# tanqiu98/2G-GCN

Measured on AMD Instinct MI355X. Metric: clips/sec fwd+bwd, T=120 N=34 C=512, higher is better.
Workload: dtype fp32

## Files before the change

2g-gcn_amd/csrc/gemm_f32.hip:

```cpp
#include <cstdlib>
#include "twog_common.h"

typedef float f32x16 __attribute__((ext_vector_type(16)));
typedef float f32x4 __attribute__((ext_vector_type(4)));

namespace {

constexpr int BK = 32;
constexpr int MAXP = 8;

struct Prob {
    twog_rows_t A, B, C;
    const float* bias;
    int M, N, K;
    int act, accumulate;
    int tiles_m, tiles_n, tile_start;
    int a_vec, b_vec;
    int n_major;
    int batch;
    int64_t a_bs, b_bs, c_bs;
    float* cs;
    int cs_acc;
};

// ... 5 lines not shown
    int cls_start[MAXP], cls_ntiles[MAXP], cls_rot[MAXP];
    int splitk;
    int k_per_split;
    int group;
    int xcd_split;
    float* slabs;
    float* cs_part;
    unsigned* xcnt;
    int xs_early;
};

struct GateArgs {
    twog_gru_step_bwd_t s[MAXP];
    float* du_part[MAXP];
    int gate_of[MAXP];
};

__device__ __forceinline__ void tile_coords(const Prob& P, int tile, int group, int& tm, int& tn) {
    const int major = P.n_major ? P.tiles_n : P.tiles_m, minor = P.n_major ? P.tiles_m : P.tiles_n;
    int a, b;
    if (group <= 1 || minor < 12) {
        a = tile / minor;
        b = tile - a * minor;
    } else {
        const int per_group = group * minor;
        const int grp = tile / per_group, first = grp * group;
        const int gsize = min(major - first, group);
        const int r = tile - grp * per_group;
        b = r / gsize;
        a = first + (r - b * gsize);
// ... 455 lines not shown
    if (kt + 1 < nkt) { split_store(r1, 1, kt + 1); __syncthreads(); compute(1); }
    if (kt + 2 < nkt) { split_store(r2, 0, kt + 2); __syncthreads(); compute(0); }
}

constexpr int X3S_RS = 4;
#ifdef TWOG_STAMPS
__device__ unsigned long long twog_stamp_buf[16 * 8];
#define TWOG_STAMP_DECL unsigned long long st_acc[6] = {0, 0, 0, 0, 0, 0}, st_last = 0; { unsigned long long t_; asm volatile("s_memtime %0\n\ts_waitcnt lgkmcnt(0)" : "=s"(t_) :: "memory"); st_last = t_; }
#define TWOG_STAMP(i) { __builtin_amdgcn_sched_barrier(0); unsigned long long t_; asm volatile("s_memtime %0\n\ts_waitcnt lgkmcnt(0)" : "=s"(t_) :: "memory"); st_acc[i] += t_ - st_last; st_last = t_; __builtin_amdgcn_sched_barrier(0); }
#define TWOG_STAMP_FLUSH if (blockIdx.x == 0 && (threadIdx.x & 63) == 0) { for (int i_ = 0; i_ < 6; ++i_) twog_stamp_buf[(threadIdx.x >> 6) * 8 + i_] = st_acc[i_]; }
#else
#define TWOG_STAMP_DECL
#define TWOG_STAMP(i)
#define TWOG_STAMP_FLUSH
#endif
template <int BM, int BN, int NT, bool BKM, int KS, int TN, bool G3, int RS = 4, bool LO2 = (TN == 1), int KU = 1>
__device__ __forceinline__ void gemm_mainloop_x3s(const twog_rows_t A, const twog_rows_t B, int M, int N, int m0, int n0,
                                                  int k_begin, int k_end, float* smem, f32x16 (&acc)[1][TN]) {
    constexpr int XK = 16 * KS, NTG = NT / KS, RB = 2 * XK;
    constexpr int WM = BM / (NTG / 128), WN = BN / 2;
    static_assert(WM == 32 && WN == 32 * TN && (!BKM || (BN == 64 && !G3)), "one 32-row block per wave, TN column blocks");
    constexpr int PA = BM * RB, PB = BN * RB, STAGE = 3 * PA + 3 * PB;
    constexpr int FA = BM * XK / 4, FB = BN * XK / 4;
    constexpr int NPA = (FA + NT - 1) / NT, NPB = (FB + NT - 1) / NT;
    static_assert(FA % NT == 0 || FA < NT, "whole passes");
    char* lds = reinterpret_cast<char*>(smem);
    TWOG_STAMP_DECL
    const int tid = threadIdx.x, lane = tid & 63, wave = (tid >> 6) % (NTG / 64), kgrp = (tid >> 6) / (NTG / 64);
    const int wm = (wave >> 1) * WM, wn = (wave & 1) * WN;
    auto swz_r = [](int row, int chunk) { return XK == 32 ? (chunk ^ ((row >> 2) & 3)) : (chunk ^ ((row >> 4) & 1)); };
    auto swz_t = [](int k, int chunk) { return chunk ^ (((k >> 1) & 1) << 2); };
// ... 12 lines not shown
    }
#pragma unroll
    for (int i = 0; i < NPB; ++i) {
        const int f = tid + i * NT;
        b_on[i] = f < FB;
        if constexpr (BKM) {
            const int kk = (f % FB) / (BN / 4), cq = f % (BN / 4);
            ob[i] = 4u * (uint32_t)((int64_t)kk * B.ld_outer + min(n0 + cq * 4, N - 4));
            sb_off[i] = 3 * PA + kk * 2 * BN + 16 * swz_t(kk, cq >> 1) + 8 * (cq & 1);
        } else {
            const int rr = (f % FB) / (XK / 4), cq = f % (XK / 4);
            int brow;
            if constexpr (G3) {
                const int gate = (rr % 96) / 32, unit = n0 + 32 * (rr / 96) + (rr & 31);
                brow = gate * N + min(unit, N - 1);
            } else {
                brow = min(n0 + rr, N - 1);
            }
            ob[i] = 4u * (uint32_t)(twog_row_off(B, brow) + cq * 4);
            sb_off[i] = 3 * PA + rr * RB + 16 * swz_r(rr, cq >> 1) + 8 * (cq & 1);
        }
    }
    struct Stage { f32x4 a[KU][NPA], b[KU][NPB]; };
    auto gload = [&](Stage& r, int k0) {
#pragma unroll
        for (int u = 0; u < KU; ++u) {
            const int sa = (int)((uint32_t)(k0 + u * XK) * 4u);
            const int sb = (int)(BKM ? (uint32_t)(k0 + u * XK) * (uint32_t)B.ld_outer * 4u : (uint32_t)(k0 + u * XK) * 4u);
#pragma unroll
            for (int i = 0; i < NPA; ++i) r.a[u][i] = __builtin_bit_cast(f32x4, __builtin_amdgcn_raw_buffer_load_b128(rsrc_a, (int)oa[i], sa, 0));
// ... 107 lines not shown
#pragma unroll
    for (int j = 0; j < RS - 1; ++j) {
        if (kt + j < nkt) {
            compute(j & 1);
            if (kt + j + 1 < nkt) { split_store(r[j + 1], (j + 1) & 1); __syncthreads(); }
        }
    }
    if constexpr (LO2) {
#pragma unroll
        for (int b = 0; b < TN; ++b)
#pragma unroll
            for (int i = 0; i < 16; ++i) acc[0][b][i] += lo[b][i];
    }
}

template <int BM, int BN, int NT, bool AKM, bool BKM, int D, bool KG, bool GATE, int KS = 1, bool XS = false, bool X3 = false, int KU = 1, bool TTMP = false>
__device__ __forceinline__ void gemm_tile(const Group& g, const GateArgs* ga) {
    constexpr int NTG = NT / KS;
    constexpr int WM = BM / (NTG / 128), WN = BN / 2;
    constexpr int TM = WM / 32, TN = WN / 32;
    constexpr int LDA = AKM ? (BM + 4) : (BK + 4);
    constexpr int LDB = BKM ? (BN + 4) : (BK + 4);
    constexpr int A_ELEMS = AKM ? BK * LDA : BM * LDA;
    constexpr int B_ELEMS = BKM ? BK * LDB : BN * LDB;
    constexpr int SMEM_FLOATS = (X3 && BM == 128 && BN == 64) ? 2 * KU * 3 * (128 + 64) * 32 / 4
                                : (X3 && BM == 128) ? 2 * X3_STAGE / 4
                                : (X3 && BM == 64 && 12 * 64 * 8 * KS * KU > 2 * (A_ELEMS + B_ELEMS)) ? 12 * 64 * 8 * KS * KU : 2 * (A_ELEMS + B_ELEMS);
    __shared__ __attribute__((aligned(16))) float smem[SMEM_FLOATS];

    int bid = 0;
    int split = blockIdx.y;
    if (!XS && g.xcd_split) {
// ... 94 lines not shown
                    const int o = (int)(((float)rowc + 0.5f) * inv_inner), i = rowc - o * inner;
                    const float* sv = S.save.ptr + (o * (int)S.save.ld_outer + i * (int)S.save.ld_inner);
                    g_dh[r] = S.dh.ptr[o * (int)S.dh.ld_outer + i * (int)S.dh.ld_inner + colc];
                    g_rg[r] = sv[colc];
                    g_z[r] = sv[H + colc];
                    g_n[r] = sv[2 * H + colc];
                    g_hn[r] = sv[3 * H + colc];
                    g_h0[r] = hp_ptr[o * hp_lo + i * hp_li + colc];
                    g_uu[r] = u_ptr[o * u_lo + i * u_li];
                }
            }
        }
    };
    const bool early = XS ? (xs_slices == 1 || g.xs_early) : !la;
    if (early) fetch_epilogue();

    const bool fast = a_vec && b_vec && ((k_end - k_begin) % BK == 0);
    if constexpr (X3) {
        if constexpr (BM == 128 && BN == 64) {
            static_assert(!X3 || BM != 128 || BN != 64 || (NT == 512 && KS == 1 && !AKM && !KG && !XS && !GATE), "X3: 128x64 chain tiles");
            gemm_mainloop_x3s<BM, BN, NT, BKM, 1, 1, false, 2, true, KU>(A, B, M, N, m0, n0, k_begin, k_end, smem, acc);
        } else if constexpr (BM == 128) {
            static_assert(!X3 || BM != 128 || (BN == 128 && NT == 512 && KS == 1 && KU == 1 && !GATE && !XS), "X3: the 8-wave 128x128 class");
            f32x4 cs = {0.f, 0.f, 0.f, 0.f};
            const bool cs_on = AKM && BKM && !KG && G.cs != nullptr && tn_idx == 0;
            gemm_mainloop_x3<AKM, BKM, KG, TTMP>(A, B, M, N, m0, n0, k_begin, k_end, smem, acc, cs, cs_on);
            if constexpr (AKM && BKM && !KG) {
                if (cs_on) {
                    __syncthreads();
                    *reinterpret_cast<f32x4*>(smem + (threadIdx.x >> 5) * 128 + (threadIdx.x & 31) * 4) = cs;
                    __syncthreads();
                    if (threadIdx.x < 128) {
                        float v = 0.f;
#pragma unroll
                        for (int r = 0; r < 16; ++r) v += smem[r * 128 + threadIdx.x];
                        const int col = m0 + (int)threadIdx.x;
                        if (g.splitk > 1) g.cs_part[((int64_t)split * g.total_tiles + bid) * 128 + threadIdx.x] = v;
                        else if (col < M) G.cs[col] = G.cs_acc ? G.cs[col] + v : v;
                    }
                    __syncthreads();
                }
            }
        } else {
            static_assert(!X3 || BM == 128 || (BM == 64 && BN == 64 && !AKM && !KG && !XS), "X3: 64x64 tiles, row-major A");
            gemm_mainloop_x3s<BM, BN, NT, BKM, KS, 1, false, (GATE || KU > 1 ? 2 : X3S_RS), true, KU>(A, B, M, N, m0, n0, k_begin, k_end, smem, acc);
        }
    } else if (fast)
        gemm_mainloop<BM, BN, NT, AKM, BKM, true, TM, TN, D, KG, KS>(A, B, M, N, a_vec, b_vec, m0, n0, k_begin, k_end, smem, acc);
    else
        gemm_mainloop<BM, BN, NT, AKM, BKM, false, TM, TN, 1, false, KS>(A, B, M, N, a_vec, b_vec, m0, n0, k_begin, k_end, smem, acc);
    if constexpr (KS == 2) {
        __syncthreads();
        float* red = smem + ((wave * TM * TN * 16) << 6) + lane;
        if (kgrp == 1) {
#pragma unroll
            for (int a = 0; a < TM; ++a)
#pragma unroll
                for (int b = 0; b < TN; ++b)
#pragma unroll
                    for (int r = 0; r < 16; ++r) red[((a * TN + b) * 16 + r) << 6] = acc[a][b][r];
        }
        __syncthreads();
        if (kgrp == 1) return;
#pragma unroll
        for (int a = 0; a < TM; ++a)
// ... 215 lines not shown

template <bool BKM, int KS>
__global__ __launch_bounds__(256 * KS, 2) void gemm_x3s_kernel(const Group g) {
    gemm_tile<64, 64, 256 * KS, false, BKM, 2, false, false, KS, false, true>(g, nullptr);
}
template <int KS>
__global__ __launch_bounds__(256 * KS, 2) void gemm_gate_bwd_x3s_kernel(const Group g, const GateArgs ga) {
    gemm_tile<64, 64, 256 * KS, false, true, 2, false, true, KS, false, true>(g, &ga);
}

template <bool BKM>
__global__ __launch_bounds__(512, 1) void gemm_x3su128_kernel(const Group g) {
    gemm_tile<128, 64, 512, false, BKM, 2, false, false, 1, false, true, 2>(g, nullptr);
}

template <bool BKM, int KS, int KU>
__global__ __launch_bounds__(256 * KS, KS == 2 ? 1 : 2) void gemm_x3su_kernel(const Group g) {
    gemm_tile<64, 64, 256 * KS, false, BKM, 2, false, false, KS, false, true, KU>(g, nullptr);
}
template <int KS, int KU>
__global__ __launch_bounds__(256 * KS, KS == 2 ? 1 : 2) void gemm_gate_bwd_x3su_kernel(const Group g, const GateArgs ga) {
    gemm_tile<64, 64, 256 * KS, false, true, 2, false, true, KS, false, true, KU>(g, &ga);
}

template <int D>
__global__ __launch_bounds__(256, 2) void gemm_gate_bwd_kernel(const Group g, const GateArgs ga) {
    gemm_tile<64, 64, 256, false, true, D, false, true>(g, &ga);
}

template <bool BKM, int D>
// ... 256 lines not shown
        hipLaunchKernelGGL((splitk_reduce_kernel<BM, BN>), dim3(g.total_tiles, (BM * BN) / 1024), dim3(256), 0, st, g);
        TWOG_CHECK_LAUNCH();
    }
    return 0;
}

thread_local int g_last_class = 0;

}

extern "C" int twog_gemm_last_class(void) { return g_last_class; }

constexpr size_t SPLITK_TICKET_BYTES = 16384;

static void prepare_group(const twog_gemm_t* pr, int n, int a_kmajor, int b_kmajor, void* workspace,
                          size_t workspace_bytes, Group& g, int* order, bool& big, int& bm) {
    int64_t tiles128 = 0;
    int kmax = 0;
    bool wide = true;
    for (int i = 0; i < n; ++i) {
        const int nb = pr[i].batch > 0 ? pr[i].batch : 1;
        tiles128 += (int64_t)nb * ((pr[i].M + 127) / 128) * ((pr[i].N + 127) / 128);
        if (pr[i].K > kmax) kmax = pr[i].K;
        if (pr[i].M < 96 || pr[i].N < 96) wide = false;
    }
    static const int force_tile = getenv("TWOG_GEMM_TILE") ? atoi(getenv("TWOG_GEMM_TILE")) : 0;
    static const int force_split = getenv("TWOG_GEMM_SPLITK") ? atoi(getenv("TWOG_GEMM_SPLITK")) : 0;
    const int64_t reach128 = tiles128 * (workspace ? (kmax >= 1024 ? kmax / 512 : 1) : 1);
    static const int big_min = getenv("TWOG_GEMM_BIG_MIN") ? atoi(getenv("TWOG_GEMM_BIG_MIN")) : 200;
    big = wide && (tiles128 >= big_min || reach128 >= 256);
    if (force_tile == 128) big = true;
    if (force_tile == 64) big = false;
    const int BMN = big ? 128 : 64;
    bm = BMN;
    {
        static const int bm32_on = getenv("TWOG_GEMM_BM32") ? atoi(getenv("TWOG_GEMM_BM32")) : 1;
        static const int ks_allowed = getenv("TWOG_GEMM_KS") ? atoi(getenv("TWOG_GEMM_KS")) : 1;
        int64_t tiles32 = 0;
        bool plain = true;
        for (int i = 0; i < n; ++i) {
            tiles32 += (int64_t)((pr[i].M + 31) / 32) * ((pr[i].N + 63) / 64);
            plain = plain && pr[i].batch <= 1 && !(b_kmajor && pr[i].B.inner > 1);
        }
        if (bm32_on && ks_allowed && !big && !a_kmajor && !workspace && plain && kmax >= 256 && tiles32 <= 256) bm = 32;
    }
// ... 193 lines not shown
    if (!any) return true;
    static const int w8 = getenv("TWOG_GEMM_W8") ? atoi(getenv("TWOG_GEMM_W8")) : 1;
    return a_kmajor && b_kmajor && big && w8 && plain && x3_128_ok(g);
}

static bool rows128_pays(const Group& g) {
    static const int on = getenv("TWOG_X3_ROWS128") ? atoi(getenv("TWOG_X3_ROWS128")) : 1;
    if (!on) return false;
    int t64 = 0, t128 = 0;
    for (int i = 0; i < g.n; ++i) {
        const Prob& P = g.p[i];
        if (P.M < 128 || P.batch > 1) return false;
        t64 += ((P.M + 63) / 64) * P.tiles_n;
        t128 += ((P.M + 127) / 128) * P.tiles_n;
    }
    if (t128 < 128 || t128 > 256) return false;
    const int c64 = ((t64 + 255) / 256) * 128, c128 = ((t128 + 255) / 256) * 192;
    return c128 * 100 <= c64 * 85;
}
static void retile_rows(Group& g, int bm) {
    int t = 0;
    g.n_cls = 0;
    for (int i = 0; i < g.n; ++i) {
        Prob& P = g.p[i];
        P.tiles_m = (P.M + bm - 1) / bm;
        P.tile_start = t;
        const int ntiles = P.batch * P.tiles_m * P.tiles_n;
        if (i == 0 || P.K != g.p[i - 1].K) {
            g.cls_start[g.n_cls] = t;
            g.cls_ntiles[g.n_cls] = 0;
            ++g.n_cls;
// ... 44 lines not shown
    if (n_problems <= 0) return 0;
    hipStream_t st = reinterpret_cast<hipStream_t>(stream);
    {
        bool any_cs = false;
        for (int i = 0; i < n_problems; ++i) any_cs = any_cs || problems[i].a_colsum != nullptr;
        if (any_cs && (chain_ws || !twog_gemm_colsum_fused(problems, n_problems, a_kmajor, b_kmajor, workspace, workspace_bytes))) return -5;
    }
    int done = 0;
    while (done < n_problems) {
        const int n = (n_problems - done) < MAXP ? (n_problems - done) : MAXP;
        const twog_gemm_t* pr = problems + done;
        Group g;
        int order[MAXP];
        bool big;
        int bm;
        prepare_group(pr, n, a_kmajor, b_kmajor, workspace, workspace_bytes, g, order, big, bm);
        static const int depth = getenv("TWOG_GEMM_DEPTH") ? atoi(getenv("TWOG_GEMM_DEPTH")) : 0;
        const int d128 = depth ? (depth & 3) : 2, d64 = depth ? ((depth >> 2) & 3) : 2;
        int rc;
        static const int w8 = getenv("TWOG_GEMM_W8") ? atoi(getenv("TWOG_GEMM_W8")) : 1;
        bool grouped = false;
        for (int i = 0; i < n; ++i) grouped = grouped || (a_kmajor && pr[i].A.inner > 1) || (b_kmajor && pr[i].B.inner > 1);
        g_last_class = (big ? TWOG_GEMM_CLASS_TILE128 : 0) | (big && w8 && !grouped ? TWOG_GEMM_CLASS_WAVES8 : 0) |
                       (grouped ? TWOG_GEMM_CLASS_KG : 0) | (g.splitk > 1 ? TWOG_GEMM_CLASS_SPLITK : 0);
        static const int ks_on = getenv("TWOG_GEMM_KS") ? atoi(getenv("TWOG_GEMM_KS")) : 1;
        int kmax_ = 0;
        for (int i = 0; i < n; ++i) kmax_ = pr[i].K > kmax_ ? pr[i].K : kmax_;
        const bool ks = ks_on && !big && !a_kmajor && !grouped && g.splitk == 1 && g.total_tiles <= 384 && kmax_ >= 256;
        if (!big && bm == 64 && !grouped && chain_ws && x3s_ok(g, a_kmajor, 32) && rows128_pays(g)) {
            retile_rows(g, 128);
            g_last_class |= TWOG_GEMM_CLASS_X3 | TWOG_GEMM_CLASS_WAVES8;
// ... 163 lines not shown
        hipLaunchKernelGGL(gemm_gate_bwd_ks_kernel<2>, grid, dim3(512), 0, (hipStream_t)stream, g, ga);
        TWOG_CHECK_LAUNCH();
        return 0;
    }
    if (x3s_ok(g, 0, 16)) {
        g_last_class |= TWOG_GEMM_CLASS_X3;
        hipLaunchKernelGGL(gemm_gate_bwd_x3s_kernel<1>, grid, block, 0, (hipStream_t)stream, g, ga);
    } else if (d64 == 2) hipLaunchKernelGGL(gemm_gate_bwd_kernel<2>, grid, block, 0, (hipStream_t)stream, g, ga);
    else hipLaunchKernelGGL(gemm_gate_bwd_kernel<1>, grid, block, 0, (hipStream_t)stream, g, ga);
    TWOG_CHECK_LAUNCH();
    return 0;
}

int twog_internal_gru_fwd_mode(void) {
    const char* e = getenv("TWOG_GRU_FWD_FUSION");
    return e ? atoi(e) : 3;
}

int twog_internal_gemm_gru_fwd(const twog_gemm_t* gh, const twog_gemm_t* gim, const twog_gru_step_t* st, int n,
                               int dry_run, void* stream) {
    const int mode = twog_internal_gru_fwd_mode();
    static const int ksplit = getenv("TWOG_GRU_FWD_KS") ? atoi(getenv("TWOG_GRU_FWD_KS")) : 2;
    const bool with_msgs = gim != nullptr;
    if (!(mode & (with_msgs ? 2 : 1)) || n <= 0 || n > MAXP) return 1;
    const int h = st[0].hidden;
    if (h < 32 || h % BK) return 1;
    auto span31 = [](const twog_rows_t& m, int rows, int64_t width) {
        const int inner = m.inner > 1 ? m.inner : 1;
        const int64_t last = (int64_t)((rows - 1) / inner) * m.ld_outer + (int64_t)((rows - 1) % inner) * (m.inner > 1 ? m.ld_inner : 0) + width;
        return m.ld_outer >= 0 && m.ld_inner >= 0 && last < (int64_t(1) << 31);
    };
// ... 45 lines not shown
    for (int i = n; i < MAXP; ++i) { g.p[i] = g.p[0]; g.p[i].rt_start = 0x7fffffff; }
    g_last_class = TWOG_GEMM_CLASS_GRUFWD;
    static const int x3_on = (getenv("TWOG_GEMM_X3") ? atoi(getenv("TWOG_GEMM_X3")) : 1) && (getenv("TWOG_GEMM_X3S") ? atoi(getenv("TWOG_GEMM_X3S")) : 1) &&
                             (getenv("TWOG_GEMM_X3G") ? atoi(getenv("TWOG_GEMM_X3G")) : 1);
    bool x3 = x3_on && ksplit == 2 && h >= 256 && h % 32 == 0;
    for (int i = 0; i < n; ++i) x3 = x3 && g.p[i].K2 % 32 == 0;
    if (x3) {
        g_last_class |= TWOG_GEMM_CLASS_X3;
        hipLaunchKernelGGL((gemm_gru_fwd_kernel<2, 2, true>), dim3(rt * g.tiles_n), dim3(512), 0, (hipStream_t)stream, g);
    } else if (ksplit == 2) hipLaunchKernelGGL((gemm_gru_fwd_kernel<2, 2>), dim3(rt * g.tiles_n), dim3(512), 0, (hipStream_t)stream, g);
    else hipLaunchKernelGGL((gemm_gru_fwd_kernel<2, 1>), dim3(rt * g.tiles_n), dim3(256), 0, (hipStream_t)stream, g);
    TWOG_CHECK_LAUNCH();
    return 0;
}

#ifdef TWOG_STAMPS
extern "C" int twog_debug_stamps(unsigned long long* out) {
    return -(int)hipMemcpyFromSymbol(out, HIP_SYMBOL(twog_stamp_buf), sizeof(unsigned long long) * 16 * 8);
}
#endif

extern "C" const char* twog_version(void) {
    return "lib2ggcn_hip gfx950 fp32 gemm on bf16x3 MFMA(32x32x16) / fp32 MFMA(32x32x2), tiles 128x128 / 64x64 / 32x64";
}
```

2g-gcn_amd/csrc/gru.hip:

```cpp
#include "twog_common.h"
#include "graph_cache.h"

namespace {

constexpr int MAXS = 8;
struct FwdGroup { twog_gru_step_t s[MAXS]; };
struct BwdGroup { twog_gru_step_bwd_t s[MAXS]; };

__device__ __forceinline__ float gate_u(const float* u, int64_t ldo, int64_t ldi, int inner, int r) {
    if (!u) return 1.0f;
    if (inner <= 1) return u[(int64_t)r * ldo];
    const int o = r / inner;
    return u[(int64_t)o * ldo + (int64_t)(r - o * inner) * ldi];
}

__device__ __forceinline__ float gru_gate_unit(float ir, float iz, float in_, float hr, float hz, float hn, float h0, bool has_u,
                                               float uu, float& rg, float& z, float& n) {
#pragma clang fp contract(off)
    rg = 1.0f / (1.0f + expf(-(ir + hr)));
    z = 1.0f / (1.0f + expf(-(iz + hz)));
    n = tanhf(fmaf(rg, hn, in_));
    const float gnew = fmaf(z, h0, (1.0f - z) * n);
    return has_u ? fmaf(uu, gnew, (1.0f - uu) * h0) : gnew;
}

__global__ __launch_bounds__(256) void gru_step_fwd_kernel(const FwdGroup g) {
    const twog_gru_step_t& S = g.s[blockIdx.y];
    const int r = blockIdx.x;
    if (r >= S.rows) return;
    const int H = S.hidden;
    const float* gi = twog_row_ptr(S.gi, r);
    const float* gi2 = S.gi2.ptr ? twog_row_ptr(S.gi2, r) : nullptr;
    const float* gh = twog_row_ptr(S.gh, r);
    const float* hp = S.h_prev.ptr ? twog_row_ptr(S.h_prev, r) : nullptr;
    float* ho = twog_row_ptr(S.h_out, r);
    float* sv = S.save.ptr ? twog_row_ptr(S.save, r) : nullptr;
    const float uu = gate_u(S.u, S.u_ld_outer, S.u_ld_inner, S.u_inner, r);
#pragma unroll 2
// ... 356 lines not shown
```

2g-gcn_amd/csrc/segrnn.hip:

```cpp
#include "twog_common.h"
#include "graph_cache.h"

namespace {

inline twog_rows_t rows_be(const float* base, int E, int64_t row_w, int T) {
    twog_rows_t r;
    r.ptr = const_cast<float*>(base); r.inner = E; r.ld_inner = row_w; r.ld_outer = (int64_t)T * E * row_w; r.pad_ = 0;
    return r;
}
inline twog_rows_t rows_plain(const float* base, int64_t ld) {
    twog_rows_t r;
    r.ptr = const_cast<float*>(base); r.inner = 1; r.ld_inner = ld; r.ld_outer = ld; r.pad_ = 0;
    return r;
}
inline twog_rows_t rows_null() {
    twog_rows_t r;
    r.ptr = nullptr; r.inner = 1; r.ld_inner = 0; r.ld_outer = 0; r.pad_ = 0;
    return r;
}
inline void gemm_set(twog_gemm_t& G, twog_rows_t A, twog_rows_t B, twog_rows_t C, const float* bias, int M, int N,
                     int K, int act, int acc) {
    G.A = A; G.B = B; G.C = C; G.bias = bias; G.M = M; G.N = N; G.K = K; G.act = act; G.accumulate = acc; G.batch = 1;
    G.a_batch_stride = G.b_batch_stride = G.c_batch_stride = 0;
    G.a_colsum = nullptr; G.a_colsum_accumulate = 0; G.pad2_ = 0;
// ... 34 lines not shown
    A.out_sh = nul; A.out_so = nul;
    A.obj_mask = S.obj_mask;
    A.att = S.att + ((int64_t)dir * d.T + t) * d.bs * d.natt;
    A.n_inst = d.bs; A.inst_per_clip = 1; A.H = d.H; A.O = d.O; A.D = h; A.hidden = h;
    A.scale = S.att_scale;
    A.recv_mask_ho = 0;
}

}

static int segrnn_fwd_impl(const twog_segrnn_t* desc, void* chain_ws, size_t chain_ws_bytes, void* stream) {
    const twog_segrnn_t& S = *desc;
    const Dims d = dims_of(S);
    const int h = d.h, T = d.T;
    const bool msg = S.msg_segment && (d.nmh + d.nmo) > 0;
    for (int s = 0; s < T; ++s) {
        const bool first = (s == 0);
        twog_gemm_t gm[8];
        int n = 0, rc;
        if (msg) {
            for (int dir = 0; dir < 2; ++dir) {
                const int t = dir == 0 ? s : T - 1 - s, tp = dir == 0 ? t - 1 : t + 1;
                if (d.nsh && d.H) {
                    twog_rows_t A = first ? rows_plain(S.zeros, h)
                                          : rows_be(S.hs_h + (int64_t)tp * d.H * 2 * h + dir * h, d.H, 2 * h, T);
                    float* C = S.msrc_h + ((int64_t)dir * d.bs * T * d.H + (int64_t)t * d.H) * d.nsh * h;
                    gemm_set(gm[n++], A, rows_plain(S.w_smsg_h, h), rows_be(C, d.H, d.nsh * h, T), S.b_smsg_h,
                             d.bs * d.H, d.nsh * h, h, 1, 0);
                }
                if (d.nso && d.O) {
                    twog_rows_t A = first ? rows_plain(S.zeros, h)
                                          : rows_be(S.hs_o + (int64_t)tp * d.O * 2 * h + dir * h, d.O, 2 * h, T);
                    float* C = S.msrc_o + ((int64_t)dir * d.bs * T * d.O + (int64_t)t * d.O) * d.nso * h;
                    gemm_set(gm[n++], A, rows_plain(S.w_smsg_o, h), rows_be(C, d.O, d.nso * h, T), S.b_smsg_o,
                             d.bs * d.O, d.nso * h, h, 1, 0);
                }
            }
            rc = twog_gemm_f32_chain(gm, n, 0, 0, chain_ws, chain_ws_bytes, stream);
            if (rc) return rc;
            twog_attn_t at[2];
            for (int dir = 0; dir < 2; ++dir) {
                const int t = dir == 0 ? s : T - 1 - s, tp = dir == 0 ? t - 1 : t + 1;
                fill_attn(at[dir], S, d, dir, t, first, tp);
            }
            rc = twog_attn_fwd(at, 2, stream);
            if (rc) return rc;
        }
        n = 0;
        twog_gru_step_t st[4];
        twog_gemm_t ghp[4], gimp[4];
        int ns = 0;
        for (int dir = 0; dir < 2; ++dir) {
            const int t = dir == 0 ? s : T - 1 - s, tp = dir == 0 ? t - 1 : t + 1;
            for (int kind = 0; kind < 2; ++kind) {
                const int E = kind == 0 ? d.H : d.O;
                if (E == 0) continue;
                const int rows = d.bs * E, nm = kind == 0 ? d.nmh : d.nmo;
                float* hs = kind == 0 ? S.hs_h : S.hs_o;
                twog_rows_t hprev = first ? rows_plain(S.zeros, h)
                                          : rows_be(hs + (int64_t)tp * E * 2 * h + dir * h, E, 2 * h, T);
                float* tmp_gh = (kind == 0 ? S.tmp_gh_h : S.tmp_gh_o) + (int64_t)dir * rows * 3 * h;
                float* tmp_gim = (kind == 0 ? S.tmp_gim_h : S.tmp_gim_o) + (int64_t)dir * rows * 3 * h;
                const float* whh = kind == 0 ? S.w_hh_h[dir] : S.w_hh_o[dir];
                const float* bhh = kind == 0 ? S.b_hh_h[dir] : S.b_hh_o[dir];
                gemm_set(gm[n], hprev, rows_plain(whh, h), rows_plain(tmp_gh, 3 * h), bhh, rows, 3 * h, h, 0, 0);
                ghp[ns] = gm[n++];
                gimp[ns].M = 0;
                if (msg && nm) {
                    const float* mg = (kind == 0 ? S.mg_h : S.mg_o) + ((int64_t)dir * d.bs * T * E + (int64_t)t * E) * nm * h;
                    const float* wim = kind == 0 ? S.w_ihm_h[dir] : S.w_ihm_o[dir];
                    const int64_t ldw = kind == 0 ? S.ld_ih_h : S.ld_ih_o;
                    gemm_set(gm[n], rows_be(mg, E, nm * h, T), rows_plain(wim, ldw), rows_plain(tmp_gim, 3 * h),
                             nullptr, rows, 3 * h, nm * h, 0, 0);
                    gimp[ns] = gm[n++];
                }
                twog_gru_step_t& G = st[ns++];
                const float* gi = kind == 0 ? S.gi_h : S.gi_o;
                G.gi = rows_be(gi + (int64_t)t * E * 6 * h + dir * 3 * h, E, 6 * h, T);
                G.gi2 = (msg && nm) ? rows_plain(tmp_gim, 3 * h) : rows_null();
                G.gh = rows_plain(tmp_gh, 3 * h);
                G.h_prev = first ? rows_null() : hprev;
                G.h_out = rows_be(hs + (int64_t)t * E * 2 * h + dir * h, E, 2 * h, T);
                float* sv = kind == 0 ? S.save_h : S.save_o;
                G.save = rows_be(sv + ((int64_t)dir * d.bs * T * E + (int64_t)t * E) * 4 * h, E, 4 * h, T);
                G.u = (kind == 0 ? S.u_h : S.u_o) + (int64_t)t * E;
                G.u_ld_outer = (int64_t)T * E; G.u_ld_inner = 1; G.u_inner = E;
                G.rows = rows; G.hidden = h;
            }
        }
        rc = twog_internal_gemm_gru_fwd(ghp, gimp, st, ns, 0, stream);
        if (rc < 0) return rc;
        if (rc == 0) continue;
        rc = twog_gemm_f32_chain(gm, n, 0, 0, chain_ws, chain_ws_bytes, stream);
        if (rc) return rc;
        rc = twog_gru_step_fwd(st, ns, stream);
        if (rc) return rc;
    }
    return 0;
}

__global__ __launch_bounds__(256) void du_reduce_kernel(const float* part, float* du, int bs, int T, int E, int P) {
    const int i = blockIdx.x * blockDim.x + threadIdx.x;
    if (i >= bs * T * E) return;
// ... 201 lines not shown
```

2g-gcn_amd/csrc/twog_common.h:

```cpp
#pragma once
#include <hip/hip_runtime.h>
#include <stdint.h>
#include <atomic>
#include "../../include/twog_gcn.h"

#define TWOG_WAVE 64

#define TWOG_CHECK_LAUNCH()                         \
    do {                                            \
        hipError_t e_ = hipGetLastError();          \
        if (e_ != hipSuccess) return -(int)e_;      \
    } while (0)

template <class K>
inline void twog_allow_dynamic_lds(K kernel, int bytes, std::atomic<uint32_t>& done) {
    int dev = 0;
    if (hipGetDevice(&dev) != hipSuccess) { (void)hipGetLastError(); dev = 0; }
    const uint32_t bit = 1u << (dev & 31);
    if (done.load(std::memory_order_acquire) & bit) return;
    (void)hipFuncSetAttribute(reinterpret_cast<const void*>(kernel), hipFuncAttributeMaxDynamicSharedMemorySize, bytes);
    done.fetch_or(bit, std::memory_order_release);
}

int twog_internal_gemm_gate_bwd(const twog_gemm_t* problems, int n, const twog_gru_step_bwd_t* gates,
                                float* const* du_part, int dry_run, void* chain_ws, size_t chain_ws_bytes, void* stream);

int twog_internal_gemm_gru_fwd(const twog_gemm_t* gh, const twog_gemm_t* gim, const twog_gru_step_t* steps, int n,
                               int dry_run, void* stream);

int twog_internal_gru_fwd_mode(void);

int twog_internal_plan_fused_fwd(int n_frames, int n_nodes, int out[4]);
int twog_internal_plan_attn2(int kernel, int n_frames, int n_nodes, int out[4]);

constexpr int TWOG_GCN_WIDE_MAX_NODES = 256;
int twog_internal_embed1_fwd_grid(int64_t rows);

inline int twog_stream_blocks(int kernel, int64_t work) {
    if (work < 0) return -2;
    int64_t items = work, cap;
    switch (kernel) {
        case TWOG_STREAM_RELU_BWD_VEC: items = work / 4; cap = 4096; break;
        case TWOG_STREAM_RELU_BWD:
// ... 31 lines not shown
    return v;
}

__device__ __forceinline__ float block_sum(float v, float* red) {
    v = wave_sum(v);
    const int lane = threadIdx.x & 63, w = threadIdx.x >> 6, nw = blockDim.x >> 6;
    __syncthreads();
    if (lane == 0) red[w] = v;
    __syncthreads();
    float t = 0.f;
    for (int i = 0; i < nw; ++i) t += red[i];
    return t;
}

__device__ __forceinline__ float sigmoidf_(float x) { return 1.0f / (1.0f + __expf(-x)); }
```

2g-gcn_amd/kernels.py:

```python
import ctypes as C
import math
import os

import torch

from . import _lib as L


def _ptr(t):
    return 0 if t is None else t.data_ptr()


_RAW_STREAM = getattr(torch._C, '_cuda_getCurrentRawStream', None)
_CUR_DEVICE = getattr(torch._C, '_cuda_getDevice', None)
if _CUR_DEVICE is None:
    _RAW_STREAM = None


def rows_of(t):
    r = L.Rows()
    if t is None:
        r.ptr, r.ld_outer, r.ld_inner, r.inner = 0, 0, 0, 1
        return r
    assert t.dtype == torch.float32, t.dtype
# ... 243 lines not shown
            self._check(rc, 'twog_gemm_f32_chain')
            return
        if self._tape is not None:
            self._tape.append((L.TAPE_GEMM, n, int(a_kmajor) | int(b_kmajor) << 1, arr))
            return
        ws_ptr, ws_bytes = 0, 0
        if split_k_workspace:
            ws = self.workspace(320 << 20, dev, 'splitk')
            ws_ptr, ws_bytes = ws.data_ptr(), ws.numel() * 4
        rc = self.lib.twog_gemm_f32(arr, n, int(a_kmajor), int(b_kmajor), ws_ptr, ws_bytes, self._stream())
        self._check(rc, 'twog_gemm_f32')

    GEMM_TILE128, GEMM_WAVES8, GEMM_KG, GEMM_SPLITK, GEMM_GATE, GEMM_KSPLIT, GEMM_GRUFWD, GEMM_ROWS32 = 1, 2, 4, 8, 16, 32, 64, 128
    GEMM_XSPLIT = 256
    GEMM_X3 = 512

    def gemm_last_class(self):
        return int(self.lib.twog_gemm_last_class())

    @staticmethod
    def _geo(x_human):
        assert x_human.is_contiguous() and x_human.dtype == torch.float32
        bs, T, H, Fh = x_human.shape
        return x_human.data_ptr() + 2048 * 4, H * Fh, bs * T

    PLAN_FUSED_FWD, PLAN_ATTN2_FWD, PLAN_ATTN2_BWD, PLAN_EMBED1_FWD, PLAN_ATTN_FWD, PLAN_ATTN_BWD = range(6)

    def gcn_launch_plan(self, kernel, n_frames, n_nodes):
        out = (C.c_int * 4)()
        self._check(self.lib.twog_gcn_launch_plan(kernel, n_frames, n_nodes, out), 'twog_gcn_launch_plan')
# ... 1084 lines not shown
```

include/twog_gcn.h:

```cpp
#ifndef TWOG_GCN_H
#define TWOG_GCN_H

#include <stddef.h>
#include <stdint.h>

#ifdef __cplusplus
extern "C" {
#endif

typedef struct {
    float* ptr;
    int64_t ld_outer;
    int64_t ld_inner;
    int32_t inner;
    int32_t pad_;
} twog_rows_t;

const char* twog_version(void);

typedef struct {
    twog_rows_t A, B, C;
    const float* bias;
    int32_t M, N, K;
    int32_t act;
// ... 7 lines not shown
int twog_gemm_f32(const twog_gemm_t* problems, int n_problems, int a_kmajor, int b_kmajor, void* workspace,
                  size_t workspace_bytes, void* stream);
int twog_gemm_colsum_fused(const twog_gemm_t* problems, int n_problems, int a_kmajor, int b_kmajor, void* workspace,
                           size_t workspace_bytes);

#define TWOG_GEMM_CLASS_TILE128 1
#define TWOG_GEMM_CLASS_WAVES8  2
#define TWOG_GEMM_CLASS_KG      4
#define TWOG_GEMM_CLASS_SPLITK  8
#define TWOG_GEMM_CLASS_GATE    16
#define TWOG_GEMM_CLASS_KSPLIT  32
#define TWOG_GEMM_CLASS_GRUFWD  64
#define TWOG_GEMM_CLASS_ROWS32  128
#define TWOG_GEMM_CLASS_XSPLIT  256
#define TWOG_GEMM_CLASS_X3      512
int twog_gemm_last_class(void);

size_t twog_chain_workspace_bytes(void);
int twog_gemm_f32_chain(const twog_gemm_t* problems, int n_problems, int a_kmajor, int b_kmajor, void* chain_ws,
                        size_t chain_ws_bytes, void* stream);

int twog_gcn_max_nodes(void);
#define TWOG_GCN_PLAN_FUSED_FWD 0
#define TWOG_GCN_PLAN_ATTN2_FWD 1
#define TWOG_GCN_PLAN_ATTN2_BWD 2
#define TWOG_GCN_PLAN_EMBED1_FWD 3
#define TWOG_GCN_PLAN_ATTN_FWD 4
#define TWOG_GCN_PLAN_ATTN_BWD 5
int twog_gcn_launch_plan(int kernel, int n_frames, int n_nodes, int out[4]);
int twog_bn_stats(const float* x_geo, int64_t frame_stride, int n_frames, int n_nodes, double* partials, int n_blocks,
// ... 483 lines not shown
```

Measured before the change: 966.5.

## Fuse GRU forward gate epilogue into message-input GEMM with gate-interleaved tiles

Adds a 128x64 X3 GEMM variant whose columns map 21 hidden units across the three gates, so the GRU gate nonlinearity runs in the GEMM epilogue and writes h_out and the saved gates directly. The hidden-to-hidden GEMMs are moved into the earlier message chain launch, and the default forward fusion mode switches so each timestep uses one fused gate launch in place of a separate input GEMM plus gate kernel. This is meant to remove a kernel launch and a round-trip of the gate pre-activations per step of the sequential recurrence. In exchange, only 63 of 64 tile columns do useful work, the epilogue adds register pressure, and the step fails hard if the fused path is refused after the dry-run check passed.

New measurement: 975.0, median of 6. About the same (+0.9%).

```diff
diff --git a/2g-gcn_amd/csrc/gemm_f32.hip b/2g-gcn_amd/csrc/gemm_f32.hip
--- a/2g-gcn_amd/csrc/gemm_f32.hip
+++ b/2g-gcn_amd/csrc/gemm_f32.hip
@@ -43,6 +43,18 @@
     twog_gru_step_bwd_t s[MAXP];
     float* du_part[MAXP];
     int gate_of[MAXP];
+};
+
+constexpr int FG_UNITS = 21;
+constexpr int FG_MAXP = 4;
+struct FGateProb {
+    twog_rows_t gi, gh, h_prev, h_out, save;
+    const float* u;
+    int u_ld_outer, u_ld_inner, inner;
+};
+struct FGateArgs {
+    FGateProb s[FG_MAXP];
+    int hidden;
 };
 
 __device__ __forceinline__ void tile_coords(const Prob& P, int tile, int group, int& tm, int& tn) {
@@ -528,7 +540,7 @@
 #define TWOG_STAMP(i)
 #define TWOG_STAMP_FLUSH
 #endif
-template <int BM, int BN, int NT, bool BKM, int KS, int TN, bool G3, int RS = 4, bool LO2 = (TN == 1), int KU = 1>
+template <int BM, int BN, int NT, bool BKM, int KS, int TN, bool G3, int RS = 4, bool LO2 = (TN == 1), int KU = 1, bool G21 = false>
 __device__ __forceinline__ void gemm_mainloop_x3s(const twog_rows_t A, const twog_rows_t B, int M, int N, int m0, int n0,
                                                   int k_begin, int k_end, float* smem, f32x16 (&acc)[1][TN]) {
     constexpr int XK = 16 * KS, NTG = NT / KS, RB = 2 * XK;
@@ -571,6 +583,10 @@
             if constexpr (G3) {
                 const int gate = (rr % 96) / 32, unit = n0 + 32 * (rr / 96) + (rr & 31);
                 brow = gate * N + min(unit, N - 1);
+            } else if constexpr (G21) {
+                static_assert(!G21 || (BN == 64 && TN == 1 && !G3), "gate-interleaved column map: 21 units x 3 gates per 64 columns");
+                const int gate = min(rr / 21, 2), unit = n0 + rr % 21;
+                brow = gate * N + min(unit, N - 1);
             } else {
                 brow = min(n0 + rr, N - 1);
             }
@@ -708,8 +724,8 @@
     }
 }
 
-template <int BM, int BN, int NT, bool AKM, bool BKM, int D, bool KG, bool GATE, int KS = 1, bool XS = false, bool X3 = false, int KU = 1, bool TTMP = false>
-__device__ __forceinline__ void gemm_tile(const Group& g, const GateArgs* ga) {
+template <int BM, int BN, int NT, bool AKM, bool BKM, int D, bool KG, bool GATE, int KS = 1, bool XS = false, bool X3 = false, int KU = 1, bool TTMP = false, bool FGATE = false>
+__device__ __forceinline__ void gemm_tile(const Group& g, const GateArgs* ga, const FGateArgs* fa = nullptr) {
     constexpr int NTG = NT / KS;
     constexpr int WM = BM / (NTG / 128), WN = BN / 2;
     constexpr int TM = WM / 32, TN = WN / 32;
@@ -834,12 +850,37 @@
     };
     const bool early = XS ? (xs_slices == 1 || g.xs_early) : !la;
     if (early) fetch_epilogue();
+    constexpr int FGP = FGATE ? (BM * FG_UNITS + NT - 1) / NT : 1;
+    float f_ir[FGP], f_iz[FGP], f_in[FGP], f_hr[FGP], f_hz[FGP], f_hn[FGP], f_h0[FGP], f_uu[FGP];
+    if constexpr (FGATE) {
+        const FGateProb& S = fa->s[pi];
+        const int H = fa->hidden, inner = S.inner;
+        const bool has_u = S.u != nullptr, has_hp = S.h_prev.ptr != nullptr;
+        const float* hp_ptr = has_hp ? S.h_prev.ptr : S.gi.ptr;
+        const int hp_lo = has_hp ? (int)S.h_prev.ld_outer : (int)S.gi.ld_outer, hp_li = has_hp ? (int)S.h_prev.ld_inner : (int)S.gi.ld_inner;
+        const float* u_ptr = has_u ? S.u : S.gi.ptr;
+        const int u_lo = has_u ? S.u_ld_outer : 0, u_li = has_u ? S.u_ld_inner : 0;
+#pragma unroll
+        for (int p = 0; p < FGP; ++p) {
+            const int item = min((int)threadIdx.x + p * NT, BM * FG_UNITS - 1);
+            const int rl = item / FG_UNITS, ul = item - rl * FG_UNITS;
+            const int rowc = min(m0 + rl, M - 1), unitc = min(tn_idx * FG_UNITS + ul, H - 1);
+            const int o = rowc / inner, i = rowc - o * inner;
+            const float* gi = S.gi.ptr + (o * (int)S.gi.ld_outer + i * (int)S.gi.ld_inner + unitc);
+            const float* gh = S.gh.ptr + (rowc * (int)S.gh.ld_outer + unitc);
+            f_ir[p] = gi[0]; f_iz[p] = gi[H]; f_in[p] = gi[2 * H];
+            f_hr[p] = gh[0]; f_hz[p] = gh[H]; f_hn[p] = gh[2 * H];
+            f_h0[p] = hp_ptr[o * hp_lo + i * hp_li + unitc];
+            f_uu[p] = u_ptr[o * u_lo + i * u_li];
+        }
+    }
 
     const bool fast = a_vec && b_vec && ((k_end - k_begin) % BK == 0);
     if constexpr (X3) {
         if constexpr (BM == 128 && BN == 64) {
-            static_assert(!X3 || BM != 128 || BN != 64 || (NT == 512 && KS == 1 && !AKM && !KG && !XS && !GATE), "X3: 128x64 chain tiles");
-            gemm_mainloop_x3s<BM, BN, NT, BKM, 1, 1, false, 2, true, KU>(A, B, M, N, m0, n0, k_begin, k_end, smem, acc);
+            static_assert(!X3 || BM != 128 || BN != 64 || (NT == 512 && KS == 1 && !AKM && !KG && !XS && !GATE && !(FGATE && BKM)), "X3: 128x64 chain tiles");
+            if constexpr (FGATE) gemm_mainloop_x3s<BM, BN, NT, false, 1, 1, false, 2, true, KU, true>(A, B, M, fa->hidden, m0, tn_idx * FG_UNITS, k_begin, k_end, smem, acc);
+            else gemm_mainloop_x3s<BM, BN, NT, BKM, 1, 1, false, 2, true, KU>(A, B, M, N, m0, n0, k_begin, k_end, smem, acc);
         } else if constexpr (BM == 128) {
             static_assert(!X3 || BM != 128 || (BN == 128 && NT == 512 && KS == 1 && KU == 1 && !GATE && !XS), "X3: the 8-wave 128x128 class");
             f32x4 cs = {0.f, 0.f, 0.f, 0.f};
@@ -869,6 +910,37 @@
         gemm_mainloop<BM, BN, NT, AKM, BKM, true, TM, TN, D, KG, KS>(A, B, M, N, a_vec, b_vec, m0, n0, k_begin, k_end, smem, acc);
     else
         gemm_mainloop<BM, BN, NT, AKM, BKM, false, TM, TN, 1, false, KS>(A, B, M, N, a_vec, b_vec, m0, n0, k_begin, k_end, smem, acc);
+    if constexpr (FGATE) {
+        static_assert(!FGATE || (X3 && BM == 128 && BN == 64 && TM * TN == 1 && !GATE), "the forward gate epilogue is written for the 128x64 chain tile");
+        constexpr int LDT = BN + 1;
+        __syncthreads();
+#pragma unroll
+        for (int r = 0; r < 16; ++r) smem[(wm + (r & 3) + 8 * (r >> 2) + 4 * kh) * LDT + wn + li] = acc[0][0][r];
+        __syncthreads();
+        const FGateProb& S = fa->s[pi];
+        const int H = fa->hidden, inner = S.inner;
+        const bool has_u = S.u != nullptr, has_hp = S.h_prev.ptr != nullptr;
+#pragma unroll
+        for (int p = 0; p < FGP; ++p) {
+            const int item = (int)threadIdx.x + p * NT;
+            const int rl = item / FG_UNITS, ul = item - rl * FG_UNITS;
+            const int row = m0 + rl, unit = tn_idx * FG_UNITS + ul;
+            if (item >= BM * FG_UNITS || row >= M || unit >= H) continue;
+            const float* t = smem + rl * LDT + ul;
+            const float ir = f_ir[p] + t[0], iz = f_iz[p] + t[FG_UNITS], in_ = f_in[p] + t[2 * FG_UNITS];
+            const float h0 = has_hp ? f_h0[p] : 0.f;
+            float rg, z, n;
+            const float hv = gru_gate_unit(ir, iz, in_, f_hr[p], f_hz[p], f_hn[p], h0, has_u, f_uu[p], rg, z, n);
+            const int o = row / inner, i = row - o * inner;
+            S.h_out.ptr[o * (int)S.h_out.ld_outer + i * (int)S.h_out.ld_inner + unit] = hv;
+            float* sv = S.save.ptr + (o * (int)S.save.ld_outer + i * (int)S.save.ld_inner + unit);
+            sv[0] = rg;
+            sv[H] = z;
+            sv[2 * H] = n;
+            sv[3 * H] = f_hn[p];
+        }
+        return;
+    }
     if constexpr (KS == 2) {
         __syncthreads();
         float* red = smem + ((wave * TM * TN * 16) << 6) + lane;
@@ -1114,6 +1186,10 @@
     gemm_tile<128, 64, 512, false, BKM, 2, false, false, 1, false, true, 2>(g, nullptr);
 }
 
+__global__ __launch_bounds__(512, 1) void gemm_fgate_x3su128_kernel(const Group g, const FGateArgs fa) {
+    gemm_tile<128, 64, 512, false, false, 2, false, false, 1, false, true, 2, false, true>(g, nullptr, &fa);
+}
+
 template <bool BKM, int KS, int KU>
 __global__ __launch_bounds__(256 * KS, KS == 2 ? 1 : 2) void gemm_x3su_kernel(const Group g) {
     gemm_tile<64, 64, 256 * KS, false, BKM, 2, false, false, KS, false, true, KU>(g, nullptr);
@@ -1400,7 +1476,7 @@
 constexpr size_t SPLITK_TICKET_BYTES = 16384;
 
 static void prepare_group(const twog_gemm_t* pr, int n, int a_kmajor, int b_kmajor, void* workspace,
-                          size_t workspace_bytes, Group& g, int* order, bool& big, int& bm) {
+                          size_t workspace_bytes, Group& g, int* order, bool& big, int& bm, bool chain = false) {
     int64_t tiles128 = 0;
     int kmax = 0;
     bool wide = true;
@@ -1414,7 +1490,8 @@
     static const int force_split = getenv("TWOG_GEMM_SPLITK") ? atoi(getenv("TWOG_GEMM_SPLITK")) : 0;
     const int64_t reach128 = tiles128 * (workspace ? (kmax >= 1024 ? kmax / 512 : 1) : 1);
     static const int big_min = getenv("TWOG_GEMM_BIG_MIN") ? atoi(getenv("TWOG_GEMM_BIG_MIN")) : 200;
-    big = wide && (tiles128 >= big_min || reach128 >= 256);
+    static const int chain_big_min = getenv("TWOG_GEMM_CHAIN_BIG_MIN") ? atoi(getenv("TWOG_GEMM_CHAIN_BIG_MIN")) : big_min;
+    big = wide && (tiles128 >= (chain ? chain_big_min : big_min) || reach128 >= 256);
     if (force_tile == 128) big = true;
     if (force_tile == 64) big = false;
     const int BMN = big ? 128 : 64;
@@ -1638,7 +1715,8 @@
         t64 += ((P.M + 63) / 64) * P.tiles_n;
         t128 += ((P.M + 127) / 128) * P.tiles_n;
     }
-    if (t128 < 128 || t128 > 256) return false;
+    static const int max_tiles = getenv("TWOG_X3_ROWS128_MAX") ? atoi(getenv("TWOG_X3_ROWS128_MAX")) : 256;
+    if (t128 < 128 || t128 > max_tiles) return false;
     const int c64 = ((t64 + 255) / 256) * 128, c128 = ((t128 + 255) / 256) * 192;
     return c128 * 100 <= c64 * 85;
 }
@@ -1713,7 +1791,7 @@
         int order[MAXP];
         bool big;
         int bm;
-        prepare_group(pr, n, a_kmajor, b_kmajor, workspace, workspace_bytes, g, order, big, bm);
+        prepare_group(pr, n, a_kmajor, b_kmajor, workspace, workspace_bytes, g, order, big, bm, chain_ws != nullptr);
         static const int depth = getenv("TWOG_GEMM_DEPTH") ? atoi(getenv("TWOG_GEMM_DEPTH")) : 0;
         const int d128 = depth ? (depth & 3) : 2, d64 = depth ? ((depth >> 2) & 3) : 2;
         int rc;
@@ -1907,7 +1985,7 @@
 
 int twog_internal_gru_fwd_mode(void) {
     const char* e = getenv("TWOG_GRU_FWD_FUSION");
-    return e ? atoi(e) : 3;
+    return e ? atoi(e) : 11;
 }
 
 int twog_internal_gemm_gru_fwd(const twog_gemm_t* gh, const twog_gemm_t* gim, const twog_gru_step_t* st, int n,
@@ -1983,6 +2061,86 @@
     return 0;
 }
 
+int twog_internal_gemm_fgate_fwd(const twog_gemm_t* gim, const twog_gru_step_t* st, int n, int dry_run, void* stream) {
+    static const int x3_on = (getenv("TWOG_GEMM_X3") ? atoi(getenv("TWOG_GEMM_X3")) : 1) && (getenv("TWOG_GEMM_X3S") ? atoi(getenv("TWOG_GEMM_X3S")) : 1);
+    if (!(twog_internal_gru_fwd_mode() & (dry_run ? 24 : 8)) || !x3_on || n <= 0 || n > FG_MAXP) return 1;
+    const int h = st[0].hidden;
+    if (h < 32 || h % 32) return 1;
+    auto span31 = [](const twog_rows_t& m, int rows, int64_t width) {
+        const int inner = m.inner > 1 ? m.inner : 1;
+        const int64_t last = (int64_t)((rows - 1) / inner) * m.ld_outer + (int64_t)((rows - 1) % inner) * (m.inner > 1 ? m.ld_inner : 0) + width;
+        return m.ld_outer >= 0 && m.ld_inner >= 0 && last < (int64_t(1) << 31);
+    };
+    int order[FG_MAXP];
+    for (int i = 0; i < n; ++i) order[i] = i;
+    for (int i = 1; i < n; ++i)
+        for (int j = i; j > 0 && gim[order[j]].K > gim[order[j - 1]].K; --j) { const int tmp = order[j]; order[j] = order[j - 1]; order[j - 1] = tmp; }
+    Group g;
+    FGateArgs fa;
+    fa.hidden = h;
+    g.n = n;
+    g.n_cls = 0;
+    int t = 0, kmax = 0;
+    for (int i = 0; i < n; ++i) {
+        const twog_gemm_t& q = gim[order[i]];
+        const twog_gru_step_t& S = st[order[i]];
+        if (S.hidden != h || S.rows < 128 || S.rows != q.M || S.rows >= (1 << 22)) return 1;
+        if (q.N != 3 * h || q.K < 256 || q.K % 32 || q.act || q.accumulate || q.bias || q.batch > 1 || q.B.inner > 1 || q.a_colsum) return 1;
+        if (!vec_ok(q.A, 0, q.K, q.M) || !vec_ok(q.B, 0, q.K, 3 * h)) return 1;
+        const int inner = S.gi.inner > 1 ? S.gi.inner : 1;
+        auto same = [&](const twog_rows_t& m) { return (m.inner > 1 ? m.inner : 1) == inner; };
+        if (!S.gi.ptr || !S.gh.ptr || !S.h_out.ptr || !S.save.ptr || S.gh.inner > 1) return 1;
+        if (!same(S.h_out) || !same(S.save) || (S.h_prev.ptr && !same(S.h_prev))) return 1;
+        if (S.u && (S.u_inner > 1 ? S.u_inner : 1) != inner) return 1;
+        if (!span31(S.gi, S.rows, 3 * h) || !span31(S.gh, S.rows, 3 * h) || !span31(S.h_out, S.rows, h) ||
+            !span31(S.save, S.rows, 4 * h) || (S.h_prev.ptr && !span31(S.h_prev, S.rows, h)))
+            return 1;
+        if (S.u && ((int64_t)((S.rows - 1) / inner) * S.u_ld_outer + (int64_t)((S.rows - 1) % inner) * S.u_ld_inner >= (int64_t(1) << 31)))
+            return 1;
+        Prob& P = g.p[i];
+        P.A = q.A; P.B = q.B; P.C = q.C; P.bias = nullptr;
+        P.M = q.M; P.N = q.N; P.K = q.K;
+        P.act = 0; P.accumulate = 0;
+        P.cs = nullptr; P.cs_acc = 0;
+        P.tiles_m = (P.M + 127) / 128;
+        P.tiles_n = (h + FG_UNITS - 1) / FG_UNITS;
+        P.tile_start = t;
+        P.batch = 1;
+        P.n_major = P.N > P.M ? 1 : 0;
+        P.a_bs = P.b_bs = P.c_bs = 0;
+        P.a_vec = P.b_vec = 1;
+        if (i == 0 || P.K != g.p[i - 1].K) {
+            g.cls_start[g.n_cls] = t;
+            g.cls_ntiles[g.n_cls] = 0;
+            ++g.n_cls;
+        }
+        g.cls_ntiles[g.n_cls - 1] += P.tiles_m * P.tiles_n;
+        t += P.tiles_m * P.tiles_n;
+        kmax = P.K > kmax ? P.K : kmax;
+        FGateProb& F = fa.s[i];
+        F.gi = S.gi; F.gh = S.gh; F.h_prev = S.h_prev; F.h_out = S.h_out; F.save = S.save;
+        F.u = S.u; F.u_ld_outer = (int)S.u_ld_outer; F.u_ld_inner = (int)S.u_ld_inner; F.inner = inner;
+    }
+    if (t > 256) return 1;
+    if (dry_run) return 0;
+    for (int i = n; i < MAXP; ++i) { g.p[i] = g.p[0]; g.p[i].tile_start = 0x7fffffff; }
+    for (int i = n; i < FG_MAXP; ++i) fa.s[i] = fa.s[0];
+    for (int c = 0, rot = 0; c < g.n_cls; ++c) {
+        g.cls_rot[c] = rot & 7;
+        rot += g.cls_ntiles[c] & 7;
+    }
+    g.total_tiles = t;
+    g.group = 0;
+    g.splitk = 1;
+    g.k_per_split = ((kmax + BK - 1) / BK) * BK;
+    g.slabs = nullptr; g.cs_part = nullptr; g.xcnt = nullptr;
+    g.xs_early = 0; g.xcd_split = 0;
+    g_last_class = TWOG_GEMM_CLASS_FGATE | TWOG_GEMM_CLASS_X3 | TWOG_GEMM_CLASS_WAVES8;
+    hipLaunchKernelGGL(gemm_fgate_x3su128_kernel, dim3(t), dim3(512), 0, (hipStream_t)stream, g, fa);
+    TWOG_CHECK_LAUNCH();
+    return 0;
+}
+
 #ifdef TWOG_STAMPS
 extern "C" int twog_debug_stamps(unsigned long long* out) {
     return -(int)hipMemcpyFromSymbol(out, HIP_SYMBOL(twog_stamp_buf), sizeof(unsigned long long) * 16 * 8);
diff --git a/2g-gcn_amd/csrc/gru.hip b/2g-gcn_amd/csrc/gru.hip
--- a/2g-gcn_amd/csrc/gru.hip
+++ b/2g-gcn_amd/csrc/gru.hip
@@ -12,16 +12,6 @@
     if (inner <= 1) return u[(int64_t)r * ldo];
     const int o = r / inner;
     return u[(int64_t)o * ldo + (int64_t)(r - o * inner) * ldi];
-}
-
-__device__ __forceinline__ float gru_gate_unit(float ir, float iz, float in_, float hr, float hz, float hn, float h0, bool has_u,
-                                               float uu, float& rg, float& z, float& n) {
-#pragma clang fp contract(off)
-    rg = 1.0f / (1.0f + expf(-(ir + hr)));
-    z = 1.0f / (1.0f + expf(-(iz + hz)));
-    n = tanhf(fmaf(rg, hn, in_));
-    const float gnew = fmaf(z, h0, (1.0f - z) * n);
-    return has_u ? fmaf(uu, gnew, (1.0f - uu) * h0) : gnew;
 }
 
 __global__ __launch_bounds__(256) void gru_step_fwd_kernel(const FwdGroup g) {
diff --git a/2g-gcn_amd/csrc/segrnn.hip b/2g-gcn_amd/csrc/segrnn.hip
--- a/2g-gcn_amd/csrc/segrnn.hip
+++ b/2g-gcn_amd/csrc/segrnn.hip
@@ -72,39 +72,13 @@
     const Dims d = dims_of(S);
     const int h = d.h, T = d.T;
     const bool msg = S.msg_segment && (d.nmh + d.nmo) > 0;
+    const int mode = twog_internal_gru_fwd_mode();
+    bool grouped = (mode & 24) && msg && d.H > 0 && d.O > 0 && d.nsh > 0 && d.nso > 0 && d.nmh > 0 && d.nmo > 0;
+    const bool fgate = (mode & 8) != 0;
     for (int s = 0; s < T; ++s) {
         const bool first = (s == 0);
         twog_gemm_t gm[8];
         int n = 0, rc;
-        if (msg) {
-            for (int dir = 0; dir < 2; ++dir) {
-                const int t = dir == 0 ? s : T - 1 - s, tp = dir == 0 ? t - 1 : t + 1;
-                if (d.nsh && d.H) {
-                    twog_rows_t A = first ? rows_plain(S.zeros, h)
-                                          : rows_be(S.hs_h + (int64_t)tp * d.H * 2 * h + dir * h, d.H, 2 * h, T);
-                    float* C = S.msrc_h + ((int64_t)dir * d.bs * T * d.H + (int64_t)t * d.H) * d.nsh * h;
-                    gemm_set(gm[n++], A, rows_plain(S.w_smsg_h, h), rows_be(C, d.H, d.nsh * h, T), S.b_smsg_h,
-                             d.bs * d.H, d.nsh * h, h, 1, 0);
-                }
-                if (d.nso && d.O) {
-                    twog_rows_t A = first ? rows_plain(S.zeros, h)
-                                          : rows_be(S.hs_o + (int64_t)tp * d.O * 2 * h + dir * h, d.O, 2 * h, T);
-                    float* C = S.msrc_o + ((int64_t)dir * d.bs * T * d.O + (int64_t)t * d.O) * d.nso * h;
-                    gemm_set(gm[n++], A, rows_plain(S.w_smsg_o, h), rows_be(C, d.O, d.nso * h, T), S.b_smsg_o,
-                             d.bs * d.O, d.nso * h, h, 1, 0);
-                }
-            }
-            rc = twog_gemm_f32_chain(gm, n, 0, 0, chain_ws, chain_ws_bytes, stream);
-            if (rc) return rc;
-            twog_attn_t at[2];
-            for (int dir = 0; dir < 2; ++dir) {
-                const int t = dir == 0 ? s : T - 1 - s, tp = dir == 0 ? t - 1 : t + 1;
-                fill_attn(at[dir], S, d, dir, t, first, tp);
-            }
-            rc = twog_attn_fwd(at, 2, stream);
-            if (rc) return rc;
-        }
-        n = 0;
         twog_gru_step_t st[4];
         twog_gemm_t ghp[4], gimp[4];
         int ns = 0;
@@ -121,16 +95,14 @@
                 float* tmp_gim = (kind == 0 ? S.tmp_gim_h : S.tmp_gim_o) + (int64_t)dir * rows * 3 * h;
                 const float* whh = kind == 0 ? S.w_hh_h[dir] : S.w_hh_o[dir];
                 const float* bhh = kind == 0 ? S.b_hh_h[dir] : S.b_hh_o[dir];
-                gemm_set(gm[n], hprev, rows_plain(whh, h), rows_plain(tmp_gh, 3 * h), bhh, rows, 3 * h, h, 0, 0);
-                ghp[ns] = gm[n++];
+                gemm_set(ghp[ns], hprev, rows_plain(whh, h), rows_plain(tmp_gh, 3 * h), bhh, rows, 3 * h, h, 0, 0);
                 gimp[ns].M = 0;
                 if (msg && nm) {
                     const float* mg = (kind == 0 ? S.mg_h : S.mg_o) + ((int64_t)dir * d.bs * T * E + (int64_t)t * E) * nm * h;
                     const float* wim = kind == 0 ? S.w_ihm_h[dir] : S.w_ihm_o[dir];
                     const int64_t ldw = kind == 0 ? S.ld_ih_h : S.ld_ih_o;
-                    gemm_set(gm[n], rows_be(mg, E, nm * h, T), rows_plain(wim, ldw), rows_plain(tmp_gim, 3 * h),
+                    gemm_set(gimp[ns], rows_be(mg, E, nm * h, T), rows_plain(wim, ldw), rows_plain(tmp_gim, 3 * h),
                              nullptr, rows, 3 * h, nm * h, 0, 0);
-                    gimp[ns] = gm[n++];
                 }
                 twog_gru_step_t& G = st[ns++];
                 const float* gi = kind == 0 ? S.gi_h : S.gi_o;
@@ -145,6 +117,60 @@
                 G.u_ld_outer = (int64_t)T * E; G.u_ld_inner = 1; G.u_inner = E;
                 G.rows = rows; G.hidden = h;
             }
+        }
+        if (grouped && first) {
+            rc = twog_internal_gemm_fgate_fwd(gimp, st, ns, 1, stream);
+            if (rc < 0) return rc;
+            grouped = rc == 0;
+        }
+        if (msg) {
+            for (int dir = 0; dir < 2; ++dir) {
+                const int t = dir == 0 ? s : T - 1 - s, tp = dir == 0 ? t - 1 : t + 1;
+                if (d.nsh && d.H) {
+                    twog_rows_t A = first ? rows_plain(S.zeros, h)
+                                          : rows_be(S.hs_h + (int64_t)tp * d.H * 2 * h + dir * h, d.H, 2 * h, T);
+                    float* C = S.msrc_h + ((int64_t)dir * d.bs * T * d.H + (int64_t)t * d.H) * d.nsh * h;
+                    gemm_set(gm[n++], A, rows_plain(S.w_smsg_h, h), rows_be(C, d.H, d.nsh * h, T), S.b_smsg_h,
+                             d.bs * d.H, d.nsh * h, h, 1, 0);
+                }
+                if (d.nso && d.O) {
+                    twog_rows_t A = first ? rows_plain(S.zeros, h)
+                                          : rows_be(S.hs_o + (int64_t)tp * d.O * 2 * h + dir * h, d.O, 2 * h, T);
+                    float* C = S.msrc_o + ((int64_t)dir * d.bs * T * d.O + (int64_t)t * d.O) * d.nso * h;
+                    gemm_set(gm[n++], A, rows_plain(S.w_smsg_o, h), rows_be(C, d.O, d.nso * h, T), S.b_smsg_o,
+                             d.bs * d.O, d.nso * h, h, 1, 0);
+                }
+            }
+            if (grouped)
+                for (int i = 0; i < ns; ++i) gm[n++] = ghp[i];
+            rc = twog_gemm_f32_chain(gm, n, 0, 0, chain_ws, chain_ws_bytes, stream);
+            if (rc) return rc;
+            twog_attn_t at[2];
+            for (int dir = 0; dir < 2; ++dir) {
+                const int t = dir == 0 ? s : T - 1 - s, tp = dir == 0 ? t - 1 : t + 1;
+                fill_attn(at[dir], S, d, dir, t, first, tp);
+            }
+            rc = twog_attn_fwd(at, 2, stream);
+            if (rc) return rc;
+        }
+        n = 0;
+        if (grouped) {
+            if (fgate) {
+                rc = twog_internal_gemm_fgate_fwd(gimp, st, ns, 0, stream);
+                if (rc < 0) return rc;
+                if (rc == 1) return -123;
+                continue;
+            }
+            for (int i = 0; i < ns; ++i) gm[n++] = gimp[i];
+            rc = twog_gemm_f32_chain(gm, n, 0, 0, chain_ws, chain_ws_bytes, stream);
+            if (rc) return rc;
+            rc = twog_gru_step_fwd(st, ns, stream);
+            if (rc) return rc;
+            continue;
+        }
+        for (int i = 0; i < ns; ++i) {
+            gm[n++] = ghp[i];
+            if (gimp[i].M > 0) gm[n++] = gimp[i];
         }
         rc = twog_internal_gemm_gru_fwd(ghp, gimp, st, ns, 0, stream);
         if (rc < 0) return rc;
diff --git a/2g-gcn_amd/csrc/twog_common.h b/2g-gcn_amd/csrc/twog_common.h
--- a/2g-gcn_amd/csrc/twog_common.h
+++ b/2g-gcn_amd/csrc/twog_common.h
@@ -27,6 +27,8 @@
 
 int twog_internal_gemm_gru_fwd(const twog_gemm_t* gh, const twog_gemm_t* gim, const twog_gru_step_t* steps, int n,
                                int dry_run, void* stream);
+
+int twog_internal_gemm_fgate_fwd(const twog_gemm_t* gim, const twog_gru_step_t* steps, int n, int dry_run, void* stream);
 
 int twog_internal_gru_fwd_mode(void);
 
@@ -88,3 +90,13 @@
 }
 
 __device__ __forceinline__ float sigmoidf_(float x) { return 1.0f / (1.0f + __expf(-x)); }
+
+__device__ __forceinline__ float gru_gate_unit(float ir, float iz, float in_, float hr, float hz, float hn, float h0, bool has_u,
+                                               float uu, float& rg, float& z, float& n) {
+#pragma clang fp contract(off)
+    rg = 1.0f / (1.0f + expf(-(ir + hr)));
+    z = 1.0f / (1.0f + expf(-(iz + hz)));
+    n = tanhf(fmaf(rg, hn, in_));
+    const float gnew = fmaf(z, h0, (1.0f - z) * n);
+    return has_u ? fmaf(uu, gnew, (1.0f - uu) * h0) : gnew;
+}
diff --git a/2g-gcn_amd/kernels.py b/2g-gcn_amd/kernels.py
--- a/2g-gcn_amd/kernels.py
+++ b/2g-gcn_amd/kernels.py
@@ -281,6 +281,7 @@
     GEMM_TILE128, GEMM_WAVES8, GEMM_KG, GEMM_SPLITK, GEMM_GATE, GEMM_KSPLIT, GEMM_GRUFWD, GEMM_ROWS32 = 1, 2, 4, 8, 16, 32, 64, 128
     GEMM_XSPLIT = 256
     GEMM_X3 = 512
+    GEMM_FGATE = 1024
 
     def gemm_last_class(self):
         return int(self.lib.twog_gemm_last_class())
diff --git a/include/twog_gcn.h b/include/twog_gcn.h
--- a/include/twog_gcn.h
+++ b/include/twog_gcn.h
@@ -45,6 +45,7 @@
 #define TWOG_GEMM_CLASS_ROWS32  128
 #define TWOG_GEMM_CLASS_XSPLIT  256
 #define TWOG_GEMM_CLASS_X3      512
+#define TWOG_GEMM_CLASS_FGATE   1024
 int twog_gemm_last_class(void);
 
 size_t twog_chain_workspace_bytes(void);
```
